# Ray0089/geometric-aware-dense-matching

Hardware: AMD Instinct MI355X
Metric: rgbd_crops_per_sec_geomatch_fwd (higher is better)
Workload: dtype bf16x3/f32acc

## Files before the change

geometric_aware_dense_matching_amd/csrc/gdm_common.h:

```cpp
#pragma once
#include <hip/hip_runtime.h>
#include <stdint.h>
#include <stdio.h>
#include <stdarg.h>
#include "../../include/gdm.h"

void gdm_set_error(const char* fmt, ...);

#define GDM_CHECK_ARG(cond, ...)                   \
    do {                                           \
        if (!(cond)) {                             \
            gdm_set_error(__VA_ARGS__);            \
            return GDM_EINVAL;                     \
        }                                          \
    } while (0)

#define GDM_HIP(call)                                                              \
    do {                                                                           \
        hipError_t _e = (call);                                                    \
        if (_e != hipSuccess) {                                                    \
            gdm_set_error("%s failed: %s", #call, hipGetErrorString(_e));          \
            return (int)_e;                                                        \
        }                                                                          \
    } while (0)

static inline int gdm_launch_status(const char* what)
{
    hipError_t e = hipGetLastError();
    if (e != hipSuccess) {
        gdm_set_error("launch of %s failed: %s", what, hipGetErrorString(e));
        return (int)e;
    }
    return 0;
}

static inline int gdm_cdiv(long a, long b) { return (int)((a + b - 1) / b); }

#ifdef __cplusplus
#include <type_traits>
template <int N, int I = 0, class F>
static inline void gdm_dispatch_int(int v, F&& f)
{
    if constexpr (I + 1 < N) {
        if (v != I) return gdm_dispatch_int<N, I + 1>(v, f);
    }
    f(std::integral_constant<int, I>{});
}
template <class F>
static inline void gdm_dispatch_bool(bool v, F&& f)
{
    if (v) f(std::true_type{});
    else f(std::false_type{});
}

template <auto Kernel>
static inline void gdm_allow_lds(int bytes)
{
    static const hipError_t once = hipFuncSetAttribute((const void*)Kernel, hipFuncAttributeMaxDynamicSharedMemorySize, bytes);
    (void)once;
}
#endif

#ifdef __HIPCC__
typedef __attribute__((ext_vector_type(2))) float gdm_f32x2;
typedef __attribute__((ext_vector_type(2))) __bf16 gdm_bf16x2;
typedef __attribute__((ext_vector_type(16))) float gdm_f32x16;
typedef __attribute__((ext_vector_type(4))) float gdm_f32x4;
typedef __attribute__((ext_vector_type(8))) __bf16 gdm_bf16x8;
typedef __attribute__((ext_vector_type(4))) unsigned gdm_u32x4;
template <int ROWB>
__device__ __forceinline__ int gdm_swz(int row, int ch) { return row * ROWB + (((ch & 16) | ((ch ^ row) & 15)) << 4); }
__device__ __forceinline__ unsigned gdm_bf16_pk(float a, float b)
{
    const gdm_f32x2 v = {a, b};
    return __builtin_bit_cast(unsigned, __builtin_convertvector(v, gdm_bf16x2));
}
__device__ __forceinline__ void gdm_split2(float a, float b, unsigned& hi, unsigned& lo)
{
    hi = gdm_bf16_pk(a, b);
    lo = gdm_bf16_pk(a - __uint_as_float(hi << 16), b - __uint_as_float(hi & 0xffff0000u));
}
__device__ __forceinline__ void gdm_split8(const float (&v)[8], gdm_u32x4& hi, gdm_u32x4& lo)
{
#pragma unroll
    for (int j = 0; j < 4; ++j) {
        unsigned h, l;
        gdm_split2(v[2 * j], v[2 * j + 1], h, l);
        hi[j] = h, lo[j] = l;
    }
// ... 5 lines not shown
```

geometric_aware_dense_matching_amd/csrc/gdm_pointwise.hip:

```cpp
#include "gdm_common.h"
#include <stdlib.h>

namespace {

constexpr int PT = 64, XS = 68;
constexpr int MAXSEG = 4;

struct PwSegDev {
    const float* x;
    const int32_t* idx;
    int C, n_src;
};

struct PwArgs {
    PwSegDev seg[MAXSEG];
    int nseg;
    const float* wt;
    long wks, wcs;
    const float* scale;
    const float* shift;
    float* out;
    int n, Cout, outC, out_c0, point_major, act, K;
    float slope;
    long total;
// ... 497 lines not shown
    }
}

bool seg_ok(const gdm_pw_seg& s, int n)
{
    return s.x && s.C >= 1 && s.n_src >= 1 && (s.idx || s.n_src == n);
}

}

extern "C" int gdm_pointwise2_hip(const gdm_pw_seg* segs, int nseg, const float* wt, int w_rowmajor, const float* scale, const float* shift,
                                  int B, int n, int Cout, int act, float slope, float* out, int out_C, int out_c0, int point_major,
                                  void* stream)
{
    GDM_CHECK_ARG(segs && wt && out, "gdm_pointwise2_hip: NULL pointer");
    GDM_CHECK_ARG(nseg >= 1 && nseg <= MAXSEG, "gdm_pointwise2_hip: nseg=%d not in [1,%d]", nseg, MAXSEG);
    GDM_CHECK_ARG(B >= 1 && n >= 1 && Cout >= 1, "gdm_pointwise2_hip: bad shape B=%d n=%d Cout=%d", B, n, Cout);
    GDM_CHECK_ARG(out_c0 >= 0 && out_c0 + Cout <= out_C, "gdm_pointwise2_hip: channels [%d, %d) outside the output's %d", out_c0,
                  out_c0 + Cout, out_C);
    GDM_CHECK_ARG(act >= 0 && act <= 2, "gdm_pointwise2_hip: act=%d", act);
    PwArgs a;
    a.K = 0;
    for (int s = 0; s < MAXSEG; ++s) {
        if (s < nseg) {
            GDM_CHECK_ARG(seg_ok(segs[s], n), "gdm_pointwise2_hip: segment %d: NULL / empty, or n_src=%d != n=%d without an index", s,
                          segs[s].n_src, n);
            a.seg[s] = PwSegDev{segs[s].x, segs[s].idx, segs[s].C, segs[s].n_src};
            a.K += segs[s].C;
        } else
            a.seg[s] = PwSegDev{nullptr, nullptr, 0, 0};
    }
    GDM_CHECK_ARG(((uintptr_t)out & 15) == 0, "gdm_pointwise2_hip: out must be 16-byte aligned");
    a.nseg = nseg;
    a.wt = wt;
    a.wks = w_rowmajor ? 1 : Cout;
    a.wcs = w_rowmajor ? a.K : 1;
    a.scale = scale;
    a.shift = shift;
    a.out = out;
    a.n = n;
    a.Cout = Cout;
    a.outC = out_C;
    a.out_c0 = out_c0;
    a.point_major = point_major ? 1 : 0;
    a.act = act;
    a.slope = slope;
    a.total = (long)B * n;
    const long tiles = (a.total + PT - 1) / PT;
    GDM_CHECK_ARG(tiles <= 0x7fffffffL, "gdm_pointwise2_hip: grid too large");
    hipStream_t st = (hipStream_t)stream;
    bool vec = (n % 4 == 0) && (Cout % 4 == 0) && (((uintptr_t)wt & 15) == 0) && !w_rowmajor;
    for (int s = 0; s < nseg; ++s) vec = vec && !segs[s].idx && (((uintptr_t)segs[s].x & 15) == 0);
    if (a.K >= 32 && gdm_cdiv(Cout, 16) <= 65535) {
        int ks = 1;
        while (ks < 8 && a.K / (2 * ks) >= 16 && tiles * gdm_cdiv(Cout, 16) * ks < 4096) ks *= 2;
        const dim3 grid((unsigned)tiles, gdm_cdiv(Cout, 16));
        bool mvec = (n % 4 == 0);
        for (int sgi = 0; sgi < nseg; ++sgi) mvec = mvec && !segs[sgi].idx && (((uintptr_t)segs[sgi].x & 15) == 0) && segs[sgi].n_src % 4 == 0;
        if (ks == 1 && Cout >= 32 && tiles >= 1024) {
            const dim3 gridc((unsigned)tiles, gdm_cdiv(Cout, 64));
            if (mvec) hipLaunchKernelGGL((pointwise_mfma_cw_kernel<true, 1>), gridc, dim3(256), 0, st, a);
            else hipLaunchKernelGGL((pointwise_mfma_cw_kernel<false, 1>), gridc, dim3(256), 0, st, a);
            return gdm_launch_status("pointwise_mfma_cw_kernel");
        }
        gdm_dispatch_int<4>(__builtin_ctz(ks), [&](auto L) {
            constexpr int KSV = 1 << decltype(L)::value;
            gdm_dispatch_bool(mvec, [&](auto V) {
                hipLaunchKernelGGL((pointwise_mfma_kernel<KSV, decltype(V)::value>), grid, dim3(KSV * 64), 0, st, a);
            });
        });
        return gdm_launch_status("pointwise_mfma_kernel");
    }
    GDM_CHECK_ARG(nseg <= 3, "gdm_pointwise2_hip: four segments need K >= 32 (the MFMA form)");
    const dim3 grid((unsigned)tiles, gdm_cdiv(Cout, 64));
    if (vec) hipLaunchKernelGGL((pointwise_kernel<4, 1, true>), grid, dim3(256), 0, st, a);
    else hipLaunchKernelGGL((pointwise_kernel<4, 1, false>), grid, dim3(256), 0, st, a);
    return gdm_launch_status("pointwise_kernel");
}

extern "C" int gdm_pointwise_jobs_hip(const gdm_pw_job* jobs, int njobs, int B, int K, int Cout, void* stream)
{
    GDM_CHECK_ARG(jobs && njobs >= 1 && njobs <= 4, "gdm_pointwise_jobs_hip: njobs=%d not in [1,4]", njobs);
    GDM_CHECK_ARG(B >= 1 && K >= 32 && Cout >= 1 && gdm_cdiv(Cout, 16) <= 65535, "gdm_pointwise_jobs_hip: bad shape B=%d K=%d Cout=%d", B, K, Cout);
    int kjob[4] = {0, 0, 0, 0};
    for (int j = 0; j < njobs; ++j) {
        const gdm_pw_job& jb = jobs[j];
        GDM_CHECK_ARG(jb.x && jb.wt && jb.out && jb.n >= 1, "gdm_pointwise_jobs_hip: job %d: NULL pointer or n=%d", j, jb.n);
        GDM_CHECK_ARG(((uintptr_t)jb.out & 15) == 0, "gdm_pointwise_jobs_hip: job %d: out must be 16-byte aligned", j);
        const long tj = ((long)B * jb.n + PT - 1) / PT;
        int kj = 1;
        while (kj < 8 && K / (2 * kj) >= 16 && tj * gdm_cdiv(Cout, 16) * kj < 4096) kj *= 2;
        kjob[j] = kj;
    }
    hipStream_t st = (hipStream_t)stream;
    for (int ks = 1; ks <= 8; ks *= 2) {
        PwArgs a[4];
        int ends[4];
        int vecmask = 0, m = 0;
        long tiles = 0;
        const gdm_pw_job* last = nullptr;
        for (int j = 0; j < njobs; ++j) {
            if (kjob[j] != ks) continue;
            const gdm_pw_job& jb = jobs[j];
            last = &jb;
            for (int sgi = 0; sgi < MAXSEG; ++sgi) a[m].seg[sgi] = PwSegDev{nullptr, nullptr, 0, 0};
            a[m].seg[0] = PwSegDev{jb.x, nullptr, K, jb.n};
            a[m].nseg = 1;
            a[m].wt = jb.wt;
            a[m].wks = Cout;
            a[m].wcs = 1;
            a[m].scale = nullptr;
            a[m].shift = nullptr;
            a[m].out = jb.out;
            a[m].n = jb.n;
            a[m].Cout = Cout;
            a[m].outC = Cout;
            a[m].out_c0 = 0;
            a[m].point_major = 0;
            a[m].act = 0;
            a[m].slope = 0.f;
            a[m].K = K;
            a[m].total = (long)B * jb.n;
            tiles += (a[m].total + PT - 1) / PT;
            if (jb.n % 4 == 0 && ((uintptr_t)jb.x & 15) == 0) vecmask |= 1 << m;
            ends[m] = (int)tiles;
            ++m;
        }
        if (m == 0) continue;
        for (int q = m; q < 4; ++q) {
            a[q] = a[m - 1];
            ends[q] = (int)tiles;
        }
        (void)last;
        GDM_CHECK_ARG(tiles <= 0x7fffffffL, "gdm_pointwise_jobs_hip: grid too large");
        const dim3 grid((unsigned)tiles, gdm_cdiv(Cout, 16));
        gdm_dispatch_int<4>(__builtin_ctz(ks), [&](auto L) {
            constexpr int KSV = 1 << decltype(L)::value;
            hipLaunchKernelGGL((pointwise_mfma_jobs_kernel<KSV>), grid, dim3(KSV * 64), 0, st, a[0], a[1], a[2], a[3], ends[0], ends[1], ends[2], vecmask);
        });
        const int rc = gdm_launch_status("pointwise_mfma_jobs_kernel");
        if (rc) return rc;
    }
    return 0;
}

// ... 17 lines not shown
```

geometric_aware_dense_matching_amd/csrc/gdm_spline.hip:

```cpp
#include "gdm_common.h"
#include "gdm_packed_act.h"
#include <math.h>

namespace {

template <bool RELU>
__global__ __launch_bounds__(128) void spline_aggregate_kernel(const float* __restrict__ xw,
                                                               const int32_t* __restrict__ rowptr,
                                                               const int32_t* __restrict__ src,
                                                               const float* __restrict__ attr,
                                                               const float* __restrict__ root,
                                                               const float* __restrict__ bias,
                                                               int C, int KS, float* __restrict__ out)
{
    const int i = blockIdx.x;
    const int nk = KS * KS * KS;
    const int e0 = rowptr[i], e1 = rowptr[i + 1];
    for (int o = threadIdx.x; o < C; o += blockDim.x) {
        float acc = 0.f;
        for (int e = e0; e < e1; ++e) {
            const int j = src[e];
            float fr[3];
            int fl[3];
#pragma unroll
// ... 248 lines not shown
constexpr int SL_RUN = 128;
#ifdef __HIP_DEVICE_COMPILE__
#define SL_NO_PACKED_F32 __attribute__((target("no-packed-fp32-ops")))
#else
#define SL_NO_PACKED_F32
#endif
template <bool RELU, int CIN_MAX>
__global__ __launch_bounds__(256) SL_NO_PACKED_F32 void spline_direct_lds_kernel(const float* __restrict__ x, const float* __restrict__ w,
                                                                const int32_t* __restrict__ rowptr, const int32_t* __restrict__ src,
                                                                const float* __restrict__ attr, const float* __restrict__ root_t,
                                                                const float* __restrict__ bias, int M, int Cin, int C, int KS,
                                                                float* __restrict__ out, float* __restrict__ out_t,
                                                                unsigned char* __restrict__ out_pk)
{
    extern __shared__ __attribute__((aligned(16))) float wl[];
    const int c0 = blockIdx.y * SL_CH;
    const int nrow = KS * KS * KS * Cin;
#pragma unroll 6
    for (int k = threadIdx.x; k < nrow * (SL_CH / 4); k += 256)
        *reinterpret_cast<float4*>(wl + 4 * k) = *reinterpret_cast<const float4*>(w + (long)(k >> 2) * C + c0 + 4 * (k & 3));
    __syncthreads();
    const int ol = (threadIdx.x & 3) * 4;
    const int i1 = min((blockIdx.x + 1) * SL_RUN, M);
    spline_rows_lds rows{wl + ol, Cin};
    for (int i = blockIdx.x * SL_RUN + (threadIdx.x >> 2); i < i1; i += 64)
        spline_direct_vertex4<RELU, CIN_MAX>(x, rows, rowptr, src, attr, root_t, bias, M, Cin, C, KS, i, c0 + ol, out, out_t, out_pk);
}

template <bool RELU>
__global__ __launch_bounds__(128) void spline_pairs_aggregate_kernel(const float* __restrict__ Y, const int32_t* __restrict__ rowptr,
                                                                     const int32_t* __restrict__ pos, const float* __restrict__ basis,
                                                                     const float* __restrict__ root, const float* __restrict__ bias,
                                                                     int C, float* __restrict__ out)
{
    const int i = blockIdx.x;
    const int e0 = rowptr[i], e1 = rowptr[i + 1];
    for (int o = threadIdx.x; o < C; o += blockDim.x) {
        float acc = 0.f;
        for (int e = e0; e < e1; ++e) {
            float m = 0.f;
#pragma unroll
            for (int s = 0; s < 8; ++s) m += basis[8 * e + s] * Y[(long)pos[8 * e + s] * C + o];
            acc += m;
        }
        const int deg = e1 - e0;
        float r = deg > 0 ? acc / (float)deg : 0.f;
        if (root) r += root[(long)i * C + o];
        if (bias) r += bias[o];
        if (RELU) r = fmaxf(r, 0.f);
        out[(long)i * C + o] = r;
    }
}

template <bool RELU>
__global__ __launch_bounds__(128) void spline_pairs_aggregate_vec_kernel(const float* __restrict__ Y, const int32_t* __restrict__ rowptr,
                                                                         const int32_t* __restrict__ pos, const float* __restrict__ basis,
                                                                         const float* __restrict__ root, const float* __restrict__ bias,
                                                                         int M, int C, float* __restrict__ out, float* __restrict__ out_t,
                                                                         unsigned char* __restrict__ out_pk)
{
    const int tpv = C / 4;
    const int i = blockIdx.x * (128 / tpv) + threadIdx.x / tpv;
    const int o = (threadIdx.x % tpv) * 4;
    if (i >= M) return;
    const int e0 = rowptr[i], e1 = rowptr[i + 1];
    float4 acc = make_float4(0.f, 0.f, 0.f, 0.f);
    for (int e = e0; e < e1; ++e) {
        float4 m = make_float4(0.f, 0.f, 0.f, 0.f);
#pragma unroll
        for (int s = 0; s < 8; ++s) {
            const float b = basis[8 * e + s];
            const float4 y = *reinterpret_cast<const float4*>(Y + (long)pos[8 * e + s] * C + o);
            m.x += b * y.x; m.y += b * y.y; m.z += b * y.z; m.w += b * y.w;
        }
        acc.x += m.x; acc.y += m.y; acc.z += m.z; acc.w += m.w;
    }
    const int deg = e1 - e0;
    float4 r = deg > 0 ? make_float4(acc.x / (float)deg, acc.y / (float)deg, acc.z / (float)deg, acc.w / (float)deg)
                       : make_float4(0.f, 0.f, 0.f, 0.f);
    if (root) {
        const float4 v = *reinterpret_cast<const float4*>(root + (long)i * C + o);
        r.x += v.x; r.y += v.y; r.z += v.z; r.w += v.w;
    }
    if (bias) {
        const float4 v = *reinterpret_cast<const float4*>(bias + o);
        r.x += v.x; r.y += v.y; r.z += v.z; r.w += v.w;
    }
    if (RELU) { r.x = fmaxf(r.x, 0.f); r.y = fmaxf(r.y, 0.f); r.z = fmaxf(r.z, 0.f); r.w = fmaxf(r.w, 0.f); }
    if (out) *reinterpret_cast<float4*>(out + (long)i * C + o) = r;
    if (out_t) {
        out_t[(long)(o + 0) * M + i] = r.x; out_t[(long)(o + 1) * M + i] = r.y;
        out_t[(long)(o + 2) * M + i] = r.z; out_t[(long)(o + 3) * M + i] = r.w;
    }
    if (out_pk) spline_store_packed(out_pk, M, i, o, r);
}

template <bool RELU>
__global__ __launch_bounds__(128) void spline_pairs_grad_kernel(const float* __restrict__ go, const float* __restrict__ out_mask,
                                                                const int32_t* __restrict__ pair_ptr, const int32_t* __restrict__ pair_ec,
                                                                const float* __restrict__ basis, const int32_t* __restrict__ tgt,
                                                                const float* __restrict__ inv_deg, int R, int C, float* __restrict__ gy,
                                                                unsigned char* __restrict__ gy_pk)
{
    const int tpv = C / 4;
    const int r = blockIdx.x * (128 / tpv) + threadIdx.x / tpv;
    const int o = (threadIdx.x % tpv) * 4;
    if (r >= R) return;
    const int q0 = pair_ptr[r], q1 = pair_ptr[r + 1];
    float4 acc = make_float4(0.f, 0.f, 0.f, 0.f);
    for (int q = q0; q < q1; ++q) {
        const int ec = pair_ec[q];
        const int t = tgt[ec >> 3];
        const float b = basis[ec] * inv_deg[t];
        float4 g = *reinterpret_cast<const float4*>(go + (long)t * C + o);
        if (RELU) {
            const float4 m = *reinterpret_cast<const float4*>(out_mask + (long)t * C + o);
            g.x = m.x > 0.f ? g.x : 0.f; g.y = m.y > 0.f ? g.y : 0.f; g.z = m.z > 0.f ? g.z : 0.f; g.w = m.w > 0.f ? g.w : 0.f;
        }
        acc.x = fmaf(b, g.x, acc.x); acc.y = fmaf(b, g.y, acc.y); acc.z = fmaf(b, g.z, acc.z); acc.w = fmaf(b, g.w, acc.w);
    }
    *reinterpret_cast<float4*>(gy + (long)r * C + o) = acc;
    if (gy_pk) spline_store_packed(gy_pk, R, r, o, acc);
}

__global__ __launch_bounds__(128) void spline_segment_sum_kernel(const float* __restrict__ z, const int32_t* __restrict__ src_ptr,
                                                                 const int32_t* __restrict__ src_rows, const float* __restrict__ add,
                                                                 int M, int C, float* __restrict__ dx)
{
    const int tpv = C / 4;
    const int j = blockIdx.x * (128 / tpv) + threadIdx.x / tpv;
    const int o = (threadIdx.x % tpv) * 4;
    if (j >= M) return;
    float4 acc = add ? *reinterpret_cast<const float4*>(add + (long)j * C + o) : make_float4(0.f, 0.f, 0.f, 0.f);
    const int q0 = src_ptr[j], q1 = src_ptr[j + 1];
    for (int q = q0; q < q1; ++q) {
        const float4 v = *reinterpret_cast<const float4*>(z + (long)src_rows[q] * C + o);
        acc.x += v.x; acc.y += v.y; acc.z += v.z; acc.w += v.w;
    }
    *reinterpret_cast<float4*>(dx + (long)j * C + o) = acc;
}


template <int CI_TILES, int NACC>
__global__ __launch_bounds__(256) void spline_wgrad_kernel(const float* __restrict__ x, const int32_t* __restrict__ rowidx,
                                                           const float* __restrict__ gy, const int32_t* __restrict__ tile_co0,
                                                           const int32_t* __restrict__ blk_start, const int32_t* __restrict__ blk_rows,
                                                           int nk, int Cin, float* __restrict__ part)
// ... 81 lines not shown

extern "C" int gdm_spline_segment_sum_hip(const float* z, const int32_t* src_ptr, const int32_t* src_rows, const float* add, int M, int C,
                                          float* dx, void* stream)
{
    GDM_CHECK_ARG(z && src_ptr && src_rows && dx, "gdm_spline_segment_sum_hip: NULL pointer");
    GDM_CHECK_ARG(M >= 1 && C >= 4 && C % 4 == 0 && C <= 512 && 512 % C == 0, "gdm_spline_segment_sum_hip: bad shape M=%d C=%d (C %% 4 == 0, 512 %% C == 0)", M, C);
    GDM_CHECK_ARG((((uintptr_t)z | (uintptr_t)add | (uintptr_t)dx) & 15) == 0, "gdm_spline_segment_sum_hip: buffers must be 16-byte aligned");
    hipLaunchKernelGGL(spline_segment_sum_kernel, dim3(gdm_cdiv(M, 128 / (C / 4))), dim3(128), 0, (hipStream_t)stream, z, src_ptr, src_rows, add, M, C, dx);
    return gdm_launch_status("spline_segment_sum_kernel");
}

extern "C" int gdm_spline_wgrad_hip(const float* x, const int32_t* rowidx, const float* gy, const int32_t* tile_co0, const int32_t* blk_start,
                                    const int32_t* blk_rows, int nk, int R, int Cin, int C, float* part, float* dw, void* stream)
{
    GDM_CHECK_ARG(x && rowidx && gy && tile_co0 && blk_start && blk_rows && part && dw, "gdm_spline_wgrad_hip: NULL pointer");
    GDM_CHECK_ARG(nk >= 1 && R >= 256 && R % 256 == 0 && C == 128 && ((Cin >= 1 && Cin <= 32) || Cin == 128),
                  "gdm_spline_wgrad_hip: nk=%d R=%d (multiple of 256) Cin=%d (<= 32 or 128) C=%d (128)", nk, R, Cin, C);
    GDM_CHECK_ARG((((uintptr_t)part | (uintptr_t)dw) & 15) == 0, "gdm_spline_wgrad_hip: part and dw must be 16-byte aligned");
    const int tiles = R / 256;
    if (Cin == 128)
        hipLaunchKernelGGL((spline_wgrad_kernel<4, 2>), dim3(tiles, 2), dim3(256), 0, (hipStream_t)stream, x, rowidx, gy, tile_co0, blk_start, blk_rows, nk, Cin, part);
    else
        hipLaunchKernelGGL((spline_wgrad_kernel<1, 1>), dim3(tiles, 1), dim3(256), 0, (hipStream_t)stream, x, rowidx, gy, tile_co0, blk_start, blk_rows, nk, Cin, part);
    const int rc = gdm_launch_status("spline_wgrad_kernel");
    if (rc != 0) return rc;
    const int per_k = Cin * C;
    hipLaunchKernelGGL(spline_wgrad_reduce_kernel, dim3(nk, gdm_cdiv(per_k, 1024)), dim3(256), 0, (hipStream_t)stream, part, blk_start, blk_rows, per_k, dw);
    return gdm_launch_status("spline_wgrad_reduce_kernel");
}

extern "C" int gdm_spline_pairs_aggregate3_hip(const float* Y, const int32_t* rowptr, const int32_t* pos, const float* basis,
                                               const float* root, const float* bias, int M, int C, int relu, float* out, float* out_t,
                                               void* out_packed, void* stream)
{
    unsigned char* out_pk = (unsigned char*)out_packed;
    GDM_CHECK_ARG(Y && rowptr && pos && basis && (out || out_t), "gdm_spline_pairs_aggregate3_hip: NULL pointer");
    GDM_CHECK_ARG(!out_pk || (C % 128 == 0 && C <= 512), "gdm_spline_pairs_aggregate3_hip: the packed output needs C = 128, 256 or 512");
    GDM_CHECK_ARG(M >= 1 && C >= 1, "gdm_spline_pairs_aggregate3_hip: bad shape");
    if (C % 4 == 0 && C <= 512 && 512 % C == 0 && ((uintptr_t)Y & 15) == 0 && ((uintptr_t)out & 15) == 0 && (!root || ((uintptr_t)root & 15) == 0) &&
        (!bias || ((uintptr_t)bias & 15) == 0)) {
        const dim3 grid(gdm_cdiv(M, 128 / (C / 4)));
        if (relu)
            hipLaunchKernelGGL(spline_pairs_aggregate_vec_kernel<true>, grid, dim3(128), 0, (hipStream_t)stream, Y, rowptr, pos, basis, root, bias, M, C, out, out_t, out_pk);
        else
            hipLaunchKernelGGL(spline_pairs_aggregate_vec_kernel<false>, grid, dim3(128), 0, (hipStream_t)stream, Y, rowptr, pos, basis, root, bias, M, C, out, out_t, out_pk);
        return gdm_launch_status("spline_pairs_aggregate_vec_kernel");
    }
    GDM_CHECK_ARG(out && !out_t && !out_pk, "gdm_spline_pairs_aggregate3_hip: the channel-major / packed outputs need C %% 4 == 0, 512 %% C == 0 and 16-byte aligned buffers");
    if (relu)
        hipLaunchKernelGGL(spline_pairs_aggregate_kernel<true>, dim3(M), dim3(128), 0, (hipStream_t)stream, Y, rowptr, pos, basis, root, bias, C, out);
    else
        hipLaunchKernelGGL(spline_pairs_aggregate_kernel<false>, dim3(M), dim3(128), 0, (hipStream_t)stream, Y, rowptr, pos, basis, root, bias, C, out);
    return gdm_launch_status("spline_pairs_aggregate_kernel");
}

extern "C" int gdm_spline_direct3_hip(const float* x, const float* weight, const int32_t* rowptr, const int32_t* src, const float* attr,
                                     const float* root_t, const float* bias, int M, int Cin, int C, int kernel_size, int relu,
                                     float* out, float* out_t, void* out_packed, int weights_in_lds, void* stream)
{
    unsigned char* out_pk = (unsigned char*)out_packed;
    GDM_CHECK_ARG(x && weight && rowptr && src && attr && (out || out_t), "gdm_spline_direct3_hip: NULL pointer");
    GDM_CHECK_ARG(!out_pk || (C % 128 == 0 && C <= 512), "gdm_spline_direct3_hip: the packed output needs C = 128, 256 or 512");
    GDM_CHECK_ARG(M >= 1 && C >= 1 && kernel_size >= 2 && Cin >= 1 && Cin <= 16, "gdm_spline_direct3_hip: bad shape M=%d Cin=%d (<= 16) C=%d ks=%d", M, Cin, C, kernel_size);
    const bool vec = C % 4 == 0 && C <= 512 && 512 % C == 0 && ((uintptr_t)weight & 15) == 0 && ((uintptr_t)out & 15) == 0 &&
                     (!root_t || ((uintptr_t)root_t & 15) == 0) && (!bias || ((uintptr_t)bias & 15) == 0);
    const int lds_bytes = 125 * Cin * SL_CH * (int)sizeof(float);
    if (vec && weights_in_lds && C == 128 && kernel_size == 5 && lds_bytes <= 160 * 1024) {
        const dim3 grid(gdm_cdiv(M, SL_RUN), C / SL_CH);
        if (relu) {
            gdm_allow_lds<spline_direct_lds_kernel<true, 16>>(125 * 16 * SL_CH * (int)sizeof(float));
            hipLaunchKernelGGL((spline_direct_lds_kernel<true, 16>), grid, dim3(256), lds_bytes, (hipStream_t)stream, x, weight, rowptr, src, attr,
                               root_t, bias, M, Cin, C, kernel_size, out, out_t, out_pk);
        } else {
            gdm_allow_lds<spline_direct_lds_kernel<false, 16>>(125 * 16 * SL_CH * (int)sizeof(float));
            hipLaunchKernelGGL((spline_direct_lds_kernel<false, 16>), grid, dim3(256), lds_bytes, (hipStream_t)stream, x, weight, rowptr, src, attr,
                               root_t, bias, M, Cin, C, kernel_size, out, out_t, out_pk);
        }
        return gdm_launch_status("spline_direct_lds_kernel");
    }
    if (vec) {
        const int vpb = 128 / (C / 4);
        const dim3 grid(gdm_cdiv(M, vpb));
        if (relu)
            hipLaunchKernelGGL((spline_direct_vec_kernel<true, 16>), grid, dim3(128), 0, (hipStream_t)stream, x, weight, rowptr, src, attr, root_t,
                               bias, M, Cin, C, kernel_size, out, out_t, out_pk);
        else
            hipLaunchKernelGGL((spline_direct_vec_kernel<false, 16>), grid, dim3(128), 0, (hipStream_t)stream, x, weight, rowptr, src, attr, root_t,
                               bias, M, Cin, C, kernel_size, out, out_t, out_pk);
        return gdm_launch_status("spline_direct_vec_kernel");
    }
    GDM_CHECK_ARG(out && !out_t && !out_pk, "gdm_spline_direct3_hip: the channel-major / packed outputs need C %% 4 == 0, 512 %% C == 0 and 16-byte aligned buffers");
    if (relu)
        hipLaunchKernelGGL((spline_direct_kernel<true, 16>), dim3(M), dim3(128), 0, (hipStream_t)stream, x, weight, rowptr, src, attr, root_t, bias, Cin, C, kernel_size, out);
    else
        hipLaunchKernelGGL((spline_direct_kernel<false, 16>), dim3(M), dim3(128), 0, (hipStream_t)stream, x, weight, rowptr, src, attr, root_t, bias, Cin, C, kernel_size, out);
    return gdm_launch_status("spline_direct_kernel");
}

extern "C" int gdm_spline_aggregate_hip(const float* xw, const int32_t* rowptr, const int32_t* src, const float* attr,
                                        const float* root, const float* bias, int M, int C, int kernel_size, int relu,
                                        float* out, void* stream)
{
    GDM_CHECK_ARG(xw && rowptr && src && attr && out, "gdm_spline_aggregate_hip: NULL pointer");
    GDM_CHECK_ARG(M >= 1 && C >= 1 && kernel_size >= 2, "gdm_spline_aggregate_hip: bad shape M=%d C=%d ks=%d", M, C, kernel_size);
    if (relu)
        hipLaunchKernelGGL(spline_aggregate_kernel<true>, dim3(M), dim3(128), 0, (hipStream_t)stream, xw, rowptr, src, attr, root, bias, C, kernel_size, out);
// ... 14 lines not shown
```

geometric_aware_dense_matching_amd/settings.py:

```python
import os


def _flag(name, default="1"):
    return os.environ.get(name, default) != "0"


USE_MFMA_CONV = _flag("GDM_MFMA_CONV")
USE_MFMA_CONV_TRAIN = _flag("GDM_MFMA_CONV_TRAIN")
USE_MFMA_GEMM = _flag("GDM_MFMA_GEMM")
USE_FUSED_UPCONV = _flag("GDM_FUSED_UPCONV")
USE_LOWRES_UPCONV_TRAIN = _flag("GDM_LOWRES_UPCONV_TRAIN")
USE_SPLIT_PSP_TRAIN = _flag("GDM_SPLIT_PSP_TRAIN")
USE_FUSED_LFA = _flag("GDM_FUSED_LFA")
USE_GROUPED_SPLINE = _flag("GDM_GROUPED_SPLINE")
USE_FUSED_BN_TRAIN = _flag("GDM_FUSED_BN_TRAIN")
USE_FUSED_SYNCBN = _flag("GDM_FUSED_SYNCBN")
USE_FUSED_MATCH_LOSS = _flag("GDM_FUSED_MATCH_LOSS")
USE_SIDE_STREAMS = _flag("GDM_SIDE_STREAMS", "0")
USE_SPARSE_FINAL = _flag("GDM_SPARSE_FINAL")
USE_FUSED_HEADS = _flag("GDM_FUSED_HEADS")
USE_MFMA_STRIDED = _flag("GDM_MFMA_STRIDED")
USE_POINTWISE = _flag("GDM_POINTWISE")
USE_OWN_STEM = _flag("GDM_OWN_STEM")
USE_GEMM_CONV1X1_TRAIN = _flag("GDM_GEMM_CONV1X1_TRAIN")
USE_MFMA_WGRAD = _flag("GDM_MFMA_WGRAD")
USE_MFMA_GEMM_TRAIN = _flag("GDM_MFMA_GEMM_TRAIN")
USE_GATHERED_FINAL = _flag("GDM_GATHERED_FINAL")
USE_DIRECT_WGRAD = _flag("GDM_DIRECT_WGRAD")
USE_FUSED_ADAM = _flag("GDM_FUSED_ADAM")
USE_POINTWISE_TRAIN = _flag("GDM_POINTWISE_TRAIN")
USE_POINT_CHAIN = _flag("GDM_POINT_CHAIN")
USE_PSP_JOBS = _flag("GDM_PSP_JOBS")
USE_PACKED_PRODUCERS = _flag("GDM_PACKED_PRODUCERS")
MESH_FORK_LATE = os.environ.get("GDM_MESH_FORK_LATE", "1") != "0"
PACK_MESH_ROWS = os.environ.get("GDM_PACK_MESH_ROWS", "1") != "0"
SPLINE_LDS_WEIGHTS = os.environ.get("GDM_SPLINE_LDS_WEIGHTS", "1") != "0"
HEADS_MATCH_ROWS = os.environ.get("GDM_HEADS_MATCH_ROWS", "1") != "0"
SIDE_PARTS = os.environ.get("GDM_SIDE_PARTS", "mesh,point,pyr").split(",")
STATIC_MATCH_ROWS = _flag("GDM_STATIC_MATCH_ROWS", "0")
UPCONV_MIN_CIN = int(os.environ.get("GDM_UPCONV_MIN_CIN", "0"))
SYNCBN_MIN_WORLD = 2

ALL_SWITCHES = ("USE_MFMA_CONV", "USE_MFMA_CONV_TRAIN", "USE_MFMA_GEMM", "USE_FUSED_UPCONV", "USE_LOWRES_UPCONV_TRAIN",
                "USE_SPLIT_PSP_TRAIN", "USE_FUSED_LFA", "USE_GROUPED_SPLINE", "USE_FUSED_BN_TRAIN", "USE_FUSED_SYNCBN",
                "USE_FUSED_MATCH_LOSS", "USE_SIDE_STREAMS", "USE_SPARSE_FINAL", "USE_FUSED_HEADS", "USE_MFMA_STRIDED", "USE_POINTWISE", "USE_OWN_STEM", "USE_GEMM_CONV1X1_TRAIN", "USE_MFMA_WGRAD", "USE_MFMA_GEMM_TRAIN", "USE_GATHERED_FINAL", "USE_DIRECT_WGRAD", "USE_PSP_JOBS", "USE_POINT_CHAIN", "USE_POINTWISE_TRAIN")
SPLIT_BF16_SWITCHES = ("USE_MFMA_CONV", "USE_MFMA_GEMM", "USE_FUSED_UPCONV", "USE_SPARSE_FINAL", "USE_FUSED_HEADS", "USE_MFMA_STRIDED",
                       "USE_OWN_STEM")
```

geometric_aware_dense_matching_amd/splinecnn.py:

```python
import os

import numpy as np
import torch
import torch.nn as nn
import torch.nn.functional as F
from torch.autograd.function import once_differentiable

from . import ops, settings
from ._lib import call
from .derived import derived
from .layers import cached_gemm_weight
from .synthetic import COLOR_MEAN, COLOR_STD_MESH

KERNEL_SIZE = 5


class _SplineAggregate(torch.autograd.Function):
    @staticmethod
    def forward(ctx, xw, root, bias, rowptr, src, attr, relu):
        M, nk, C = xw.shape
        out = torch.empty((M, C), dtype=torch.float32, device=xw.device)
        call("gdm_spline_aggregate_hip", xw, rowptr, src, attr, root, bias, M, C, KERNEL_SIZE, int(relu), out)
        ctx.save_for_backward(rowptr, src, attr, out)
        ctx.relu = relu
# ... 102 lines not shown
        R = pairs["rowidx"].shape[0]
        gy, pk = _pairs_grad(go, out, pairs, ctx.relu, ctx.needs_input_grad[0])
        g = go * (out > 0).to(go.dtype) if ctx.relu else go
        dx = None
        if ctx.needs_input_grad[0]:
            wpk = _train_gemm_weight(conv, "dgrad", weight, lambda w: w.reshape(nk * conv.cin, conv.cout))
            Z = torch.empty((R, conv.cin), dtype=torch.float32, device=x.device)
            call("gdm_gemm_grouped_hip", pk, wpk, pairs["rowid"], pairs["tile_co0"], R, R, conv.cout, nk * conv.cin, Z)
            add = g @ lin_weight
            dx = torch.empty((M, conv.cin), dtype=torch.float32, device=x.device)
            call("gdm_spline_segment_sum_hip", Z, pairs["src_ptr"], pairs["src_rows"], add, M, conv.cin, dx)
        dw = _spline_wgrad(x, gy, pairs, conv.cin, conv.cout)
        return dx, dw, g.t() @ x, g.sum(dim=0), None, None, None, None


class SplineConv(nn.Module):

    def __init__(self, cin, cout):
        super().__init__()
        self.cin, self.cout = cin, cout
        self.weight = nn.Parameter(torch.empty(KERNEL_SIZE ** 3, cin, cout))
        self.lin = nn.Linear(cin, cout, bias=False)
        self.bias = nn.Parameter(torch.zeros(cout))
        bound = 1.0 / np.sqrt(cin * KERNEL_SIZE ** 3)
        nn.init.uniform_(self.weight, -bound, bound)
        nn.init.uniform_(self.lin.weight, -bound, bound)

    def _load_from_state_dict(self, state_dict, prefix, *args, **kwargs):
        old = prefix + "root"
        if old in state_dict and prefix + "lin.weight" not in state_dict:
            state_dict[prefix + "lin.weight"] = state_dict.pop(old).t().contiguous()
        super()._load_from_state_dict(state_dict, prefix, *args, **kwargs)

    def _root_t(self):
        return derived(self, "root_t", (self.lin.weight,), lambda: self.lin.weight.t().contiguous())

    def forward_direct_cm(self, x, rowptr, src, attr, relu):
        return self.forward_direct_cm_packed(x, rowptr, src, attr, relu, False)[0]

    def forward_direct_cm_packed(self, x, rowptr, src, attr, relu, want_packed):
        M = x.shape[0]
        out_t = torch.empty((1, self.cout, M), dtype=torch.float32, device=x.device)
        pk = ops.spline_packed_buffer(self.cout, M, x.device) if want_packed and ops.spline_packed_supported(self.cout) else None
        xc = x.contiguous()
        call("gdm_spline_direct3_hip", xc, self.weight, rowptr, src, attr, self._root_t(), self.bias, M, self.cin, self.cout, KERNEL_SIZE,
             int(relu), None, out_t, pk, int(settings.SPLINE_LDS_WEIGHTS))
        return out_t, pk

    def forward_grouped_cm(self, xt, rowptr, pairs, relu, xpk=None, want_packed=False):
        M = xt.shape[2]
        nk = KERNEL_SIZE ** 3
        wpk, _ = cached_gemm_weight(self, "dense", lambda: self.weight.permute(0, 2, 1).reshape(nk * self.cout, self.cin), (self.weight,))
        Y = ops.gemm_grouped(xt, wpk, pairs["rowidx"], pairs["tile_co0"], nk * self.cout, xpk=xpk)
        root = ops.pointwise([xt], self._root_t(), point_major=True)
        out_t = torch.empty((1, self.cout, M), dtype=torch.float32, device=xt.device)
        pk = ops.spline_packed_buffer(self.cout, M, xt.device, avoid=xpk) if want_packed and ops.spline_packed_supported(self.cout) else None
        call("gdm_spline_pairs_aggregate3_hip", Y, rowptr, pairs["pos"], pairs["basis"], root, self.bias, M, self.cout, int(relu), None,
             out_t, pk)
        return out_t, pk

    def train_grouped_ok(self, x, pairs):
        if not (x.is_cuda and pairs is not None and "inv_deg" in pairs and self.cout == 128 and self.lin.bias is None):
            return False
        if self.cin <= 16:
            return not x.requires_grad
        return self.cin == 128 and settings.USE_MFMA_GEMM and settings.USE_GROUPED_SPLINE

    def forward_train_grouped(self, x, rowptr, src, attr, relu, pairs):
        x = x.contiguous()
        if self.cin <= 16:
            return _SplineDirectTrain.apply(x, self.weight, self.lin.weight, self.bias, self, rowptr, src, attr, pairs, relu)
        return _SplineGroupedTrain.apply(x, self.weight, self.lin.weight, self.bias, self, rowptr, pairs, relu)

    def forward(self, x, rowptr, src, attr, relu=False, pairs=None):
        M = x.shape[0]
        nk = KERNEL_SIZE ** 3
        if self.cin <= 16 and x.is_cuda and not torch.is_grad_enabled():
            out = torch.empty((M, self.cout), dtype=torch.float32, device=x.device)
            xc = x.contiguous()
            call("gdm_spline_direct3_hip", xc, self.weight, rowptr, src, attr, self._root_t(), self.bias, M, self.cin, self.cout,
                 KERNEL_SIZE, int(relu), out, None, None, int(settings.SPLINE_LDS_WEIGHTS))
            return out
        if (settings.USE_MFMA_GEMM and settings.USE_GROUPED_SPLINE and pairs is not None and not torch.is_grad_enabled() and x.is_cuda
                and self.cin % 128 == 0 and self.cout == 128):
            wpk, _ = cached_gemm_weight(self, "dense", lambda: self.weight.permute(0, 2, 1).reshape(nk * self.cout, self.cin),
                                        (self.weight,))
            xt = x.t().contiguous().unsqueeze(0)
            Y = ops.gemm_grouped(xt, wpk, pairs["rowidx"], pairs["tile_co0"], nk * self.cout)
            if settings.USE_POINTWISE and self.lin.bias is None:
                root = ops.pointwise([xt], self._root_t(), point_major=True).view(M, self.cout)
            else:
                root = self.lin(x)
            out = torch.empty((M, self.cout), dtype=torch.float32, device=x.device)
            call("gdm_spline_pairs_aggregate3_hip", Y, rowptr, pairs["pos"], pairs["basis"], root, self.bias, M, self.cout, int(relu), out,
                 None, None)
            return out
        if (settings.USE_MFMA_GEMM and not torch.is_grad_enabled() and x.is_cuda
                and ops.gemm_supported(self.cin, nk * self.cout, M, 1)):
            wpk, _ = cached_gemm_weight(self, "dense", lambda: self.weight.permute(0, 2, 1).reshape(nk * self.cout, self.cin),
                                        (self.weight,))
            xw = ops.gemm_bf16x3(x.t().contiguous().unsqueeze(0), wpk, nk * self.cout, pixel_major=True).view(M, nk, self.cout)
            root = self.lin(x)
            return _SplineAggregate.apply(xw, root, self.bias, rowptr, src, attr, relu)
        w = self.weight.permute(1, 0, 2).reshape(self.cin, -1)
        xw = torch.matmul(x, w).view(M, KERNEL_SIZE ** 3, self.cout)
        root = self.lin(x)
        return _SplineAggregate.apply(xw, root, self.bias, rowptr, src, attr, relu)


def mesh_node_features(model_pts):
    rgb = model_pts[:, 3:6].astype(np.uint8).astype(np.float64) / 255.0
    rgb = (rgb - COLOR_MEAN.astype(np.float64)) / COLOR_STD_MESH.astype(np.float64)
# ... 214 lines not shown
```

include/gdm.h:

```cpp
#ifndef GDM_H
#define GDM_H

#include <stddef.h>
#include <stdint.h>

#ifdef __cplusplus
extern "C" {
#endif

#define GDM_EINVAL (-1)
#define GDM_ENOMEM (-2)

const char* gdm_last_error(void);
int gdm_version(void);


void gdm_knn_batch(const float* batch_data, size_t batch_size, size_t npts, size_t dim,
                   const float* queries, size_t nqueries, size_t K, long* batch_indices);

int gdm_knn_batch_hip(const float* support, const float* query, int B, int S, int Q, int K,
                      int32_t* idx, float* d2, void* stream);

typedef struct gdm_knn_job {
    const float* support;
// ... 40 lines not shown
int gdm_att_pool_bwd_hip(const float* att, const float* feat, const float* grad_out, int B, int C, int n, int K,
                         float* grad_att, float* grad_feat, void* stream);


#define GDM_MATCH_BF16X3 0
#define GDM_MATCH_F32    1

size_t gdm_match_workspace_bytes(int B, int N, int M);

int gdm_match_hip(const float* scene, const float* model, int B, int D, int N, int M, int precision,
                  int32_t* best_idx, float* best_sim, float* sim,
                  void* workspace, size_t workspace_bytes, void* stream);

size_t gdm_match_rows_bytes(int rows);
size_t gdm_match_partial_bytes(int B, int N);
int gdm_match_pack_hip(const float* x, int R, int D, int n, int precision, void* rows, void* stream);
int gdm_match_pack2_hip(const float* x1, int R1, int n1, void* rows1, const float* x2, int R2, int n2, void* rows2,
                        int D, int precision, void* stream);
int gdm_match_packed_hip(const void* scene_rows, const void* model_rows, int R , int M, int precision,
                         int32_t* best_idx, float* best_sim, float* sim,
                         void* partial, size_t partial_bytes, void* stream);

#define GDM_MATCH_SOFT_MAX_GAMMA 40.0f
#define GDM_MATCH_SOFT_MAX_M     16384
size_t gdm_match_soft_partial_bytes(int B, int N);
int gdm_match_soft_packed_hip(const void* scene_rows, const void* model_rows, const float* model_xyz, int R , int M,
                              int precision, float gamma, int32_t* best_idx, float* best_sim, float* lse, float* conf,
                              float* soft_xyz, void* partial, size_t partial_bytes, void* stream);
int gdm_match_score_hip(const float* conf, const uint8_t* mask, int B, int N, float* score, void* stream);

size_t gdm_match_twoway_partial_bytes(int B, int N, int M);
int gdm_match_twoway_packed_hip(const void* scene_rows, const void* model_rows, const uint8_t* mask, int B, int N, int M, int precision,
                                int32_t* best_idx, float* best_sim, int32_t* col_idx, float* col_sim, void* partial,
                                size_t partial_bytes, void* stream);
int gdm_match_cycle_hip(const float* scene_xyz, long scene_bstride, int pt_stride, int ch_stride, const int32_t* best_idx,
                        const int32_t* col_idx, const uint8_t* mask, int B, int N, int M, float radius, uint8_t* pair_mask,
                        int32_t* pair_count, float* cycle_d2, void* stream);

int gdm_seg_mask_hip(const float* seg, int B, int N, uint8_t* mask, int32_t* count, void* stream);

int gdm_spline_aggregate_hip(const float* xw, const int32_t* rowptr, const int32_t* src, const float* attr,
                             const float* root, const float* bias, int M, int C, int kernel_size, int relu,
                             float* out, void* stream);
int gdm_spline_aggregate_bwd_hip(const float* grad_out, const int32_t* rowptr, const int32_t* src, const float* attr,
                                 int M, int C, int kernel_size, float* grad_xw, void* stream);
int gdm_spline_direct3_hip(const float* x, const float* weight, const int32_t* rowptr, const int32_t* src, const float* attr,
                           const float* root_t, const float* bias, int M, int Cin, int C, int kernel_size, int relu,
                           float* out, float* out_t, void* out_packed, int weights_in_lds, void* stream);
int gdm_gemm_grouped_hip(const void* xpk, const void* wpk, const int32_t* rowidx, const int32_t* tile_co0, int R, int M,
                         int Cin, int Cout_total, float* out, void* stream);
int gdm_spline_pairs_aggregate3_hip(const float* Y, const int32_t* rowptr, const int32_t* pos, const float* basis,
                                    const float* root, const float* bias, int M, int C, int relu, float* out, float* out_t,
                                    void* out_packed, void* stream);
int gdm_spline_pairs_grad_hip(const float* grad_out, const float* out_mask, const int32_t* pair_ptr, const int32_t* pair_ec,
                              const float* basis, const int32_t* tgt, const float* inv_deg, int R, int C, float* gy,
                              void* gy_packed, void* stream);
int gdm_spline_segment_sum_hip(const float* z, const int32_t* src_ptr, const int32_t* src_rows, const float* add, int M, int C,
                               float* dx, void* stream);
int gdm_spline_wgrad_hip(const float* x, const int32_t* rowidx, const float* gy, const int32_t* tile_co0, const int32_t* blk_start,
                         const int32_t* blk_rows, int nk, int R, int Cin, int C, float* part, float* dw, void* stream);

int gdm_upsample_bilinear_hip(const float* in, long planes, int H, int W, int OH, int OW, float* out, void* stream);
int gdm_upsample_bilinear_bwd_hip(const float* grad_out, long planes, int H, int W, int OH, int OW, float* grad_in, void* stream);

int gdm_topk_rows_hip(const float* score, long rows, int n, int K, int32_t* idx, float* val, void* stream);
int gdm_topk_negdist_hip(const float* gram, const float* xx, int B, int n, int K, int32_t* idx, void* stream);
int gdm_edge_feature_hip(const float* x, const int32_t* idx, int B, int C, int n, int K, float* out, void* stream);
int gdm_edge_feature_bwd_hip(const float* grad_out, const int32_t* idx, int B, int C, int n, int K, float* grad_x, void* stream);
size_t gdm_feature_knn_workspace_bytes(int B, int n);
int gdm_feature_knn_hip(const float* x, long x_bstride, int B, int C, int n, int K, int splits, void* ws, size_t ws_bytes, int32_t* idx,
                        float* val, void* stream);
int gdm_edge_block_hip(const float* pq, const int32_t* idx, const float* scale1, const float* shift1, const float* w2, const float* scale2,
                       const float* shift2, float slope, int B, int n, int K, float* out, int out_C, int out_c0, void* stream);
long gdm_edge_train_groups(int B, int n);
int gdm_edge_stats_hip(const float* pq, const int32_t* idx, const float* st1, const float* w2, float slope, int B, int n, int K, double* part,
                       void* stream);
int gdm_edge_bwd_reduce_hip(const float* pq, const int32_t* idx, const float* st1, const float* w2, const float* st2, float slope, int B, int n,
                            int K, const float* grad_out, uint8_t* amax, double* part, void* stream);
int gdm_edge_bwd_mid_hip(const float* pq, const int32_t* idx, const float* st1, const float* w2, const float* st2, const float* cf2, float slope,
                         int B, int n, int K, const float* grad_out, const uint8_t* amax, double* part, float* dw_slabs, void* stream);
int gdm_edge_bwd_scatter_hip(const float* pq, const int32_t* idx, const float* st1, const float* cf1, const float* w2, const float* st2,
                             const float* cf2, float slope, int B, int n, int K, const float* grad_out, const uint8_t* amax, float* grad_pq,
                             void* stream);

int gdm_circle_rows_fwd_hip(const float* sim, int R, int Mp, const int32_t* match, const int32_t* item,
                            const float* xyz, const uint8_t* vis, float radius, float gamma, float m,
                            float* lse_p, float* lse_n, float* loss, void* stream);
int gdm_circle_rows_bwd_hip(const float* sim, int R, int Mp, const int32_t* match, const int32_t* item,
                            const float* xyz, const uint8_t* vis, float radius, float gamma, float m,
                            const float* lse_p, const float* lse_n, const float* grad_rows, float* dsim, void* stream);

size_t gdm_circle_match_rows_bytes(int n);
size_t gdm_circle_match_tp_bytes(int n);
int gdm_circle_match_pack_hip(const float* x, int n, void* rows, void* tp, float* rowsum, void* stream);
int gdm_circle_match_nbr_hip(const float* xyz, int M, float radius, uint32_t* nbr, void* stream);
int gdm_circle_match_visbits_hip(const uint8_t* vis, int B, int M, uint32_t* bits, void* stream);
int gdm_circle_match_nbr_items_hip(const float* xyz, int M, const float* rad , int B, uint32_t* nbr, void* stream);
int gdm_circle_match_fwd2_hip(const void* xrows, const void* xtp, const float* xpad, const void* yrows, const void* ytp,
                              int R, int M, const int32_t* g, const int32_t* c2, const int32_t* item,
                              const uint32_t* nbr, int nbr_per_item, const uint32_t* visb, int pad_e0, float gamma, float m,
                              float* lse_p, float* lse_n, float* loss, void* stream);
int gdm_circle_match_bwd2_hip(const void* xrows, const void* xtp, const float* xpad, const void* yrows, const void* ytp,
                              int R, int M, const int32_t* g, const int32_t* c2, const int32_t* item,
                              const uint32_t* nbr, int nbr_per_item, const uint32_t* visb, int pad_e0, float gamma, float m,
                              const float* lse_p, const float* lse_n, const float* coef, float* gx, float* gy_part, void* stream);
int gdm_circle_match_bwd_parts(int R, int M);
// ... 287 lines not shown
```

Baseline: 5340.

## Fuse spline root linear transform into pairs aggregation kernel

Adds a kernel that computes the root linear term (xt times root_t) inside the spline pairs aggregation, so the separate pointwise launch and its intermediate root buffer are no longer needed. Each 1024-thread block stages the 128x128 root weights and a 32-point input tile in LDS and does the small matmul with FMAs alongside the gather-mean. It is used by default for inference with 128-channel layers. The trade-offs are scalar FMA in place of the MFMA pointwise path, and roughly 80KB of LDS per block, which limits occupancy.

```diff
diff --git a/geometric_aware_dense_matching_amd/csrc/gdm_common.h b/geometric_aware_dense_matching_amd/csrc/gdm_common.h
--- a/geometric_aware_dense_matching_amd/csrc/gdm_common.h
+++ b/geometric_aware_dense_matching_amd/csrc/gdm_common.h
@@ -35,6 +35,13 @@
 }
 
 static inline int gdm_cdiv(long a, long b) { return (int)((a + b - 1) / b); }
+
+static inline int gdm_pw_k_split(int K, int Cout, long tiles)
+{
+    int ks = 1;
+    while (ks < 8 && K / (2 * ks) >= 16 && tiles * gdm_cdiv(Cout, 16) * ks < 4096) ks *= 2;
+    return ks;
+}
 
 #ifdef __cplusplus
 #include <type_traits>
diff --git a/geometric_aware_dense_matching_amd/csrc/gdm_pointwise.hip b/geometric_aware_dense_matching_amd/csrc/gdm_pointwise.hip
--- a/geometric_aware_dense_matching_amd/csrc/gdm_pointwise.hip
+++ b/geometric_aware_dense_matching_amd/csrc/gdm_pointwise.hip
@@ -573,8 +573,7 @@
     bool vec = (n % 4 == 0) && (Cout % 4 == 0) && (((uintptr_t)wt & 15) == 0) && !w_rowmajor;
     for (int s = 0; s < nseg; ++s) vec = vec && !segs[s].idx && (((uintptr_t)segs[s].x & 15) == 0);
     if (a.K >= 32 && gdm_cdiv(Cout, 16) <= 65535) {
-        int ks = 1;
-        while (ks < 8 && a.K / (2 * ks) >= 16 && tiles * gdm_cdiv(Cout, 16) * ks < 4096) ks *= 2;
+        const int ks = gdm_pw_k_split(a.K, Cout, tiles);
         const dim3 grid((unsigned)tiles, gdm_cdiv(Cout, 16));
         bool mvec = (n % 4 == 0);
         for (int sgi = 0; sgi < nseg; ++sgi) mvec = mvec && !segs[sgi].idx && (((uintptr_t)segs[sgi].x & 15) == 0) && segs[sgi].n_src % 4 == 0;
@@ -609,9 +608,7 @@
         GDM_CHECK_ARG(jb.x && jb.wt && jb.out && jb.n >= 1, "gdm_pointwise_jobs_hip: job %d: NULL pointer or n=%d", j, jb.n);
         GDM_CHECK_ARG(((uintptr_t)jb.out & 15) == 0, "gdm_pointwise_jobs_hip: job %d: out must be 16-byte aligned", j);
         const long tj = ((long)B * jb.n + PT - 1) / PT;
-        int kj = 1;
-        while (kj < 8 && K / (2 * kj) >= 16 && tj * gdm_cdiv(Cout, 16) * kj < 4096) kj *= 2;
-        kjob[j] = kj;
+        kjob[j] = gdm_pw_k_split(K, Cout, tj);
     }
     hipStream_t st = (hipStream_t)stream;
     for (int ks = 1; ks <= 8; ks *= 2) {
diff --git a/geometric_aware_dense_matching_amd/csrc/gdm_spline.hip b/geometric_aware_dense_matching_amd/csrc/gdm_spline.hip
--- a/geometric_aware_dense_matching_amd/csrc/gdm_spline.hip
+++ b/geometric_aware_dense_matching_amd/csrc/gdm_spline.hip
@@ -324,6 +324,43 @@
     }
 }
 
+__device__ __forceinline__ float4 spline_pairs_mean4(const float* __restrict__ Y, const int32_t* __restrict__ rowptr,
+                                                     const int32_t* __restrict__ pos, const float* __restrict__ basis, int C, int i, int o)
+{
+    const int e0 = rowptr[i], e1 = rowptr[i + 1];
+    float4 acc = make_float4(0.f, 0.f, 0.f, 0.f);
+    for (int e = e0; e < e1; ++e) {
+        float4 m = make_float4(0.f, 0.f, 0.f, 0.f);
+#pragma unroll
+        for (int s = 0; s < 8; ++s) {
+            const float b = basis[8 * e + s];
+            const float4 y = *reinterpret_cast<const float4*>(Y + (long)pos[8 * e + s] * C + o);
+            m.x += b * y.x; m.y += b * y.y; m.z += b * y.z; m.w += b * y.w;
+        }
+        acc.x += m.x; acc.y += m.y; acc.z += m.z; acc.w += m.w;
+    }
+    const int deg = e1 - e0;
+    return deg > 0 ? make_float4(acc.x / (float)deg, acc.y / (float)deg, acc.z / (float)deg, acc.w / (float)deg)
+                   : make_float4(0.f, 0.f, 0.f, 0.f);
+}
+
+template <bool RELU>
+__device__ __forceinline__ void spline_pairs_finish4(float4 r, const float* __restrict__ bias, int M, int C, int i, int o,
+                                                     float* __restrict__ out, float* __restrict__ out_t, unsigned char* __restrict__ out_pk)
+{
+    if (bias) {
+        const float4 v = *reinterpret_cast<const float4*>(bias + o);
+        r.x += v.x; r.y += v.y; r.z += v.z; r.w += v.w;
+    }
+    if (RELU) { r.x = fmaxf(r.x, 0.f); r.y = fmaxf(r.y, 0.f); r.z = fmaxf(r.z, 0.f); r.w = fmaxf(r.w, 0.f); }
+    if (out) *reinterpret_cast<float4*>(out + (long)i * C + o) = r;
+    if (out_t) {
+        out_t[(long)(o + 0) * M + i] = r.x; out_t[(long)(o + 1) * M + i] = r.y;
+        out_t[(long)(o + 2) * M + i] = r.z; out_t[(long)(o + 3) * M + i] = r.w;
+    }
+    if (out_pk) spline_store_packed(out_pk, M, i, o, r);
+}
+
 template <bool RELU>
 __global__ __launch_bounds__(128) void spline_pairs_aggregate_vec_kernel(const float* __restrict__ Y, const int32_t* __restrict__ rowptr,
                                                                          const int32_t* __restrict__ pos, const float* __restrict__ basis,
@@ -335,36 +372,65 @@
     const int i = blockIdx.x * (128 / tpv) + threadIdx.x / tpv;
     const int o = (threadIdx.x % tpv) * 4;
     if (i >= M) return;
-    const int e0 = rowptr[i], e1 = rowptr[i + 1];
-    float4 acc = make_float4(0.f, 0.f, 0.f, 0.f);
-    for (int e = e0; e < e1; ++e) {
-        float4 m = make_float4(0.f, 0.f, 0.f, 0.f);
-#pragma unroll
-        for (int s = 0; s < 8; ++s) {
-            const float b = basis[8 * e + s];
-            const float4 y = *reinterpret_cast<const float4*>(Y + (long)pos[8 * e + s] * C + o);
-            m.x += b * y.x; m.y += b * y.y; m.z += b * y.z; m.w += b * y.w;
-        }
-        acc.x += m.x; acc.y += m.y; acc.z += m.z; acc.w += m.w;
-    }
-    const int deg = e1 - e0;
-    float4 r = deg > 0 ? make_float4(acc.x / (float)deg, acc.y / (float)deg, acc.z / (float)deg, acc.w / (float)deg)
-                       : make_float4(0.f, 0.f, 0.f, 0.f);
+    float4 r = spline_pairs_mean4(Y, rowptr, pos, basis, C, i, o);
     if (root) {
         const float4 v = *reinterpret_cast<const float4*>(root + (long)i * C + o);
         r.x += v.x; r.y += v.y; r.z += v.z; r.w += v.w;
     }
-    if (bias) {
-        const float4 v = *reinterpret_cast<const float4*>(bias + o);
-        r.x += v.x; r.y += v.y; r.z += v.z; r.w += v.w;
-    }
-    if (RELU) { r.x = fmaxf(r.x, 0.f); r.y = fmaxf(r.y, 0.f); r.z = fmaxf(r.z, 0.f); r.w = fmaxf(r.w, 0.f); }
-    if (out) *reinterpret_cast<float4*>(out + (long)i * C + o) = r;
-    if (out_t) {
-        out_t[(long)(o + 0) * M + i] = r.x; out_t[(long)(o + 1) * M + i] = r.y;
-        out_t[(long)(o + 2) * M + i] = r.z; out_t[(long)(o + 3) * M + i] = r.w;
-    }
-    if (out_pk) spline_store_packed(out_pk, M, i, o, r);
+    spline_pairs_finish4<RELU>(r, bias, M, C, i, o, out, out_t, out_pk);
+}
+
+constexpr int RA_C = 128, RA_V = 32, RA_XS = RA_C + 4;
+constexpr int RA_LDS = (RA_C * RA_C + RA_V * RA_XS) * (int)sizeof(float);
+template <bool RELU>
+__global__ __launch_bounds__(1024) SL_NO_PACKED_F32 void spline_pairs_root_aggregate_kernel(
+    const float* __restrict__ Y, const int32_t* __restrict__ rowptr, const int32_t* __restrict__ pos, const float* __restrict__ basis,
+    const float* __restrict__ xt, const float* __restrict__ root_t, const float* __restrict__ bias, int M, int ks,
+    float* __restrict__ out, float* __restrict__ out_t, unsigned char* __restrict__ out_pk)
+{
+    extern __shared__ __attribute__((aligned(16))) float ra_lds[];
+    float* const wl = ra_lds;
+    float* const xs = ra_lds + RA_C * RA_C;
+    const int tid = threadIdx.x;
+    const int v = tid >> 5, o = (tid & 31) * 4;
+    const int i0 = blockIdx.x * RA_V, i = i0 + v;
+    float4 wreg[4];
+    float xreg[4];
+#pragma unroll
+    for (int j = 0; j < 4; ++j) {
+        wreg[j] = reinterpret_cast<const float4*>(root_t)[tid + 1024 * j];
+        const int idx = tid + 1024 * j;
+        xreg[j] = xt[(long)(idx >> 5) * M + min(i0 + (idx & 31), M - 1)];
+    }
+    float4 r = make_float4(0.f, 0.f, 0.f, 0.f);
+    if (i < M) r = spline_pairs_mean4(Y, rowptr, pos, basis, RA_C, i, o);
+#pragma unroll
+    for (int j = 0; j < 4; ++j) {
+        const int idx = tid + 1024 * j;
+        reinterpret_cast<float4*>(wl)[idx] = wreg[j];
+        xs[(idx & 31) * RA_XS + (idx >> 5)] = xreg[j];
+    }
+    __syncthreads();
+    if (i >= M) return;
+    const int kpart = RA_C / ks;
+    float4 tot = make_float4(0.f, 0.f, 0.f, 0.f);
+    for (int j = 0; j < ks; ++j) {
+        float4 p = make_float4(0.f, 0.f, 0.f, 0.f);
+        for (int k = j * kpart; k < (j + 1) * kpart; k += 4) {
+            const float4 x4 = *reinterpret_cast<const float4*>(xs + v * RA_XS + k);
+            const float xk[4] = {x4.x, x4.y, x4.z, x4.w};
+#pragma unroll
+            for (int u = 0; u < 4; ++u) {
+                const float4 w4 = *reinterpret_cast<const float4*>(wl + (k + u) * RA_C + o);
+                p.x = fmaf(xk[u], w4.x, p.x); p.y = fmaf(xk[u], w4.y, p.y);
+                p.z = fmaf(xk[u], w4.z, p.z); p.w = fmaf(xk[u], w4.w, p.w);
+            }
+        }
+        if (j == 0) tot = p;
+        else { tot.x += p.x; tot.y += p.y; tot.z += p.z; tot.w += p.w; }
+    }
+    r.x += fmaf(tot.x, 1.f, 0.f); r.y += fmaf(tot.y, 1.f, 0.f); r.z += fmaf(tot.z, 1.f, 0.f); r.w += fmaf(tot.w, 1.f, 0.f);
+    spline_pairs_finish4<RELU>(r, bias, M, RA_C, i, o, out, out_t, out_pk);
 }
 
 template <bool RELU>
@@ -552,6 +618,30 @@
     else
         hipLaunchKernelGGL(spline_pairs_aggregate_kernel<false>, dim3(M), dim3(128), 0, (hipStream_t)stream, Y, rowptr, pos, basis, root, bias, C, out);
     return gdm_launch_status("spline_pairs_aggregate_kernel");
+}
+
+extern "C" int gdm_spline_pairs_root_aggregate_hip(const float* Y, const int32_t* rowptr, const int32_t* pos, const float* basis,
+                                                   const float* xt, const float* root_t, const float* bias, int M, int C, int relu,
+                                                   float* out, float* out_t, void* out_packed, void* stream)
+{
+    unsigned char* out_pk = (unsigned char*)out_packed;
+    GDM_CHECK_ARG(Y && rowptr && pos && basis && xt && root_t && (out || out_t), "gdm_spline_pairs_root_aggregate_hip: NULL pointer");
+    GDM_CHECK_ARG(M >= 1 && C == RA_C, "gdm_spline_pairs_root_aggregate_hip: built for C = Cin = 128, got M=%d C=%d", M, C);
+    GDM_CHECK_ARG((((uintptr_t)Y | (uintptr_t)root_t | (uintptr_t)bias | (uintptr_t)out | (uintptr_t)out_pk) & 15) == 0 &&
+                  (((uintptr_t)xt | (uintptr_t)out_t) & 3) == 0,
+                  "gdm_spline_pairs_root_aggregate_hip: Y, root_t, bias, out and out_packed must be 16-byte aligned (xt, out_t: 4)");
+    const int ks = gdm_pw_k_split(RA_C, RA_C, gdm_cdiv(M, 64));
+    const dim3 grid(gdm_cdiv(M, RA_V));
+    if (relu) {
+        gdm_allow_lds<spline_pairs_root_aggregate_kernel<true>>(RA_LDS);
+        hipLaunchKernelGGL(spline_pairs_root_aggregate_kernel<true>, grid, dim3(1024), RA_LDS, (hipStream_t)stream, Y, rowptr, pos, basis, xt,
+                           root_t, bias, M, ks, out, out_t, out_pk);
+    } else {
+        gdm_allow_lds<spline_pairs_root_aggregate_kernel<false>>(RA_LDS);
+        hipLaunchKernelGGL(spline_pairs_root_aggregate_kernel<false>, grid, dim3(1024), RA_LDS, (hipStream_t)stream, Y, rowptr, pos, basis, xt,
+                           root_t, bias, M, ks, out, out_t, out_pk);
+    }
+    return gdm_launch_status("spline_pairs_root_aggregate_kernel");
 }
 
 extern "C" int gdm_spline_direct3_hip(const float* x, const float* weight, const int32_t* rowptr, const int32_t* src, const float* attr,
diff --git a/geometric_aware_dense_matching_amd/settings.py b/geometric_aware_dense_matching_amd/settings.py
--- a/geometric_aware_dense_matching_amd/settings.py
+++ b/geometric_aware_dense_matching_amd/settings.py
@@ -36,6 +36,7 @@
 PACK_MESH_ROWS = os.environ.get("GDM_PACK_MESH_ROWS", "1") != "0"
 SPLINE_LDS_WEIGHTS = os.environ.get("GDM_SPLINE_LDS_WEIGHTS", "1") != "0"
 HEADS_MATCH_ROWS = os.environ.get("GDM_HEADS_MATCH_ROWS", "1") != "0"
+SPLINE_ROOT_IN_AGGREGATE = os.environ.get("GDM_SPLINE_ROOT_IN_AGGREGATE", "1") != "0"
 SIDE_PARTS = os.environ.get("GDM_SIDE_PARTS", "mesh,point,pyr").split(",")
 STATIC_MATCH_ROWS = _flag("GDM_STATIC_MATCH_ROWS", "0")
 UPCONV_MIN_CIN = int(os.environ.get("GDM_UPCONV_MIN_CIN", "0"))
diff --git a/geometric_aware_dense_matching_amd/splinecnn.py b/geometric_aware_dense_matching_amd/splinecnn.py
--- a/geometric_aware_dense_matching_amd/splinecnn.py
+++ b/geometric_aware_dense_matching_amd/splinecnn.py
@@ -178,12 +178,20 @@
         nk = KERNEL_SIZE ** 3
         wpk, _ = cached_gemm_weight(self, "dense", lambda: self.weight.permute(0, 2, 1).reshape(nk * self.cout, self.cin), (self.weight,))
         Y = ops.gemm_grouped(xt, wpk, pairs["rowidx"], pairs["tile_co0"], nk * self.cout, xpk=xpk)
-        root = ops.pointwise([xt], self._root_t(), point_major=True)
         out_t = torch.empty((1, self.cout, M), dtype=torch.float32, device=xt.device)
         pk = ops.spline_packed_buffer(self.cout, M, xt.device, avoid=xpk) if want_packed and ops.spline_packed_supported(self.cout) else None
+        if self.root_in_aggregate(xt):
+            call("gdm_spline_pairs_root_aggregate_hip", Y, rowptr, pairs["pos"], pairs["basis"], xt, self._root_t(), self.bias, M,
+                 self.cout, int(relu), None, out_t, pk)
+            return out_t, pk
+        root = ops.pointwise([xt], self._root_t(), point_major=True)
         call("gdm_spline_pairs_aggregate3_hip", Y, rowptr, pairs["pos"], pairs["basis"], root, self.bias, M, self.cout, int(relu), None,
              out_t, pk)
         return out_t, pk
+
+    def root_in_aggregate(self, xt):
+        return (settings.SPLINE_ROOT_IN_AGGREGATE and self.cin == 128 and self.cout == 128 and self.lin.bias is None
+                and not torch.is_grad_enabled() and xt.dtype == torch.float32 and xt.is_contiguous())
 
     def train_grouped_ok(self, x, pairs):
         if not (x.is_cuda and pairs is not None and "inv_deg" in pairs and self.cout == 128 and self.lin.bias is None):
diff --git a/include/gdm.h b/include/gdm.h
--- a/include/gdm.h
+++ b/include/gdm.h
@@ -116,6 +116,9 @@
 int gdm_spline_pairs_aggregate3_hip(const float* Y, const int32_t* rowptr, const int32_t* pos, const float* basis,
                                     const float* root, const float* bias, int M, int C, int relu, float* out, float* out_t,
                                     void* out_packed, void* stream);
+int gdm_spline_pairs_root_aggregate_hip(const float* Y, const int32_t* rowptr, const int32_t* pos, const float* basis,
+                                        const float* xt, const float* root_t, const float* bias, int M, int C, int relu,
+                                        float* out, float* out_t, void* out_packed, void* stream);
 int gdm_spline_pairs_grad_hip(const float* grad_out, const float* out_mask, const int32_t* pair_ptr, const int32_t* pair_ec,
                               const float* basis, const int32_t* tgt, const float* inv_deg, int R, int C, float* gy,
                               void* gy_packed, void* stream);
```

After: 5310. About the same (-0.6%).
